# PKU-VCL-Geometry/GeoSplatting

Hardware: AMD Instinct MI355X
Metric: fwd+bwd views/sec at 2M Gaussians, 800x800 (higher is better)
Workload: dtype f32

## Files before the change

### geosplatting_amd/csrc/gs_segsort_dev.h

```cpp
#pragma once
#include <stdint.h>

#ifndef GS_SEGSORT_FN
#define GS_SEGSORT_FN __device__ __forceinline__
#endif

typedef unsigned long long gs_u64;

template <bool PAD>
GS_SEGSORT_FN int gs_seg_phys(int i) { return PAD ? i + (i >> 5) : i; }

template <bool F64>
GS_SEGSORT_FN gs_u64 gs_seg_inf() { return F64 ? 0x7ff0000000000000ull : ~0ull; }

template <bool F64>
GS_SEGSORT_FN void gs_seg_cx(gs_u64& a, gs_u64& b)
{
#if defined(__HIP_DEVICE_COMPILE__)
    if (F64) {
        const double x = __builtin_bit_cast(double, a), y = __builtin_bit_cast(double, b);
        double lo, hi;
        asm("v_min_f64 %0, %1, %2" : "=v"(lo) : "v"(x), "v"(y));
        asm("v_max_f64 %0, %1, %2" : "=v"(hi) : "v"(x), "v"(y));
        a = __builtin_bit_cast(gs_u64, lo); b = __builtin_bit_cast(gs_u64, hi);
        return;
    }
#endif
    const gs_u64 lo = a < b ? a : b, hi = a < b ? b : a;
    a = lo; b = hi;
}

template <int F, bool PAD, bool F64, bool GUARD>
GS_SEGSORT_FN void gs_seg_first(gs_u64* buf, int n, int P, int tid, int nthreads)
{
    constexpr int R = 1 << F;
    for (int v = tid; v < (P >> F); v += nthreads) {
        const int base = v << F;
        if (base >= n) break;
        gs_u64 e[R];
#pragma unroll
        for (int r = 0; r < R; ++r) e[r] = (!GUARD || base + r < n) ? buf[gs_seg_phys<PAD>(base + r)] : gs_seg_inf<F64>();
#pragma unroll
        for (int lgk = 1; lgk <= F; ++lgk) {
#pragma unroll
            for (int r = 0; r < R; ++r)
                if (r < (r ^ ((1 << lgk) - 1))) gs_seg_cx<F64>(e[r], e[r ^ ((1 << lgk) - 1)]);
#pragma unroll
            for (int s = lgk - 2; s >= 0; --s) {
#pragma unroll
                for (int r = 0; r < R; ++r)
                    if ((r & (1 << s)) == 0) gs_seg_cx<F64>(e[r], e[r | (1 << s)]);
            }
        }
#pragma unroll
        for (int r = 0; r < R; ++r) if (!GUARD || base + r < n) buf[gs_seg_phys<PAD>(base + r)] = e[r];
    }
}

template <int G, bool PAD, bool F64, bool GUARD>
GS_SEGSORT_FN void gs_seg_group(gs_u64* buf, int n, int P, int a, bool flip, int tid, int nthreads)
{
    constexpr int R = 1 << G, H = R >> 1;
    const int jmask = (1 << a) - 1;
    for (int v = tid; v < (P >> G); v += nthreads) {
        const int base = ((v >> a) << (a + G)) | (v & jmask);
        if (base >= n) break;
        const int base2 = flip ? (base ^ jmask) : base;
        gs_u64 e[R];
#pragma unroll
        for (int r = 0; r < R; ++r) {
            const int i = (r >= H ? base2 : base) + (r << a);
            e[r] = (!GUARD || i < n) ? buf[gs_seg_phys<PAD>(i)] : gs_seg_inf<F64>();
        }
        if (flip) {
#pragma unroll
            for (int r = 0; r < H; ++r) gs_seg_cx<F64>(e[r], e[R - 1 - r]);
        } else {
#pragma unroll
            for (int r = 0; r < H; ++r) gs_seg_cx<F64>(e[r], e[r + H]);
        }
#pragma unroll
        for (int s = G - 2; s >= 0; --s) {
#pragma unroll
            for (int r = 0; r < R; ++r)
                if ((r & (1 << s)) == 0) gs_seg_cx<F64>(e[r], e[r | (1 << s)]);
        }
#pragma unroll
        for (int r = 0; r < R; ++r) {
            const int i = (r >= H ? base2 : base) + (r << a);
            if (!GUARD || i < n) buf[gs_seg_phys<PAD>(i)] = e[r];
        }
    }
}

template <int GMAX, bool PAD, bool F64, bool GUARD>
GS_SEGSORT_FN void gs_seg_group_n(int g, gs_u64* buf, int n, int P, int a, bool flip, int tid, int nthreads)
{
    if (g == GMAX) gs_seg_group<GMAX, PAD, F64, GUARD>(buf, n, P, a, flip, tid, nthreads);
    else if constexpr (GMAX > 1) gs_seg_group_n<GMAX - 1, PAD, F64, GUARD>(g, buf, n, P, a, flip, tid, nthreads);
}

#define GS_SEG_SORT_BODY(GMAX, PAD, F64, GUARD, buf, n, P, tid, nthreads, BARRIER)                           \
    do {                                                                                                     \
        gs_seg_first<GMAX, PAD, F64, GUARD>(buf, n, P, tid, nthreads);                                       \
        BARRIER;                                                                                             \
        for (int k_ = 2 << (GMAX), lgk_ = (GMAX) + 1; k_ <= (P); k_ <<= 1, ++lgk_) {                         \
            int rem_ = lgk_;                                                                                 \
            bool flip_ = true;                                                                               \
            while (rem_ > 0) {                                                                               \
                const int g_ = flip_ ? ((rem_ - 1) % (GMAX)) + 1 : (GMAX);                                   \
                gs_seg_group_n<GMAX, PAD, F64, GUARD>(g_, buf, n, P, rem_ - g_, flip_, tid, nthreads);       \
                BARRIER;                                                                                     \
                rem_ -= g_;                                                                                  \
                flip_ = false;                                                                               \
            }                                                                                                \
        }                                                                                                    \
    } while (0)
```

### geosplatting_amd/csrc/gs_sort.hip

```cpp
#include "gs_common.h"
#include "gs_segsort_dev.h"

#include <cstdlib>
#include <cstring>

#define RS_THREADS 256
#define RS_WAVES 4
#define RS_ITEMS 8
#define RS_TILE (RS_THREADS * RS_ITEMS)
#define RS_WCHUNK (64 * RS_ITEMS)

typedef unsigned long long u64;

static int tile_bits(int tile_w, int tile_h)
{
    unsigned n = (unsigned)(tile_w * tile_h);
    int b = 0;
    while (n > 1) { n >>= 1; ++b; }
    return b + 1;
}

struct PairItem { u64 key; int32_t val; };
struct PairIn {
    const u64* keys; const int32_t* vals;
    __device__ __forceinline__ PairItem load(int64_t i) const { return PairItem{ keys[i], vals[i] }; }
};
struct PairOut {
    u64* keys; int32_t* vals;
    __device__ __forceinline__ void store(int64_t i, const PairItem& it) const { keys[i] = it.key; vals[i] = it.val; }
};
struct PairDigit {
    int shift; unsigned mask;
    __device__ __forceinline__ unsigned operator()(const PairItem& it) const { return (unsigned)(it.key >> shift) & mask; }
};

struct U2In {
    const uint2* p;
    __device__ __forceinline__ uint2 load(int64_t i) const { return p[i]; }
};
struct U2Out {
    uint2* p;
    __device__ __forceinline__ void store(int64_t i, const uint2& it) const { p[i] = it; }
};
struct DepthIn {
    const float* depths;
    __device__ __forceinline__ uint2 load(int64_t i) const { return make_uint2(__float_as_uint(depths[i]), (unsigned)i); }
};
struct XDigit {
    int shift; unsigned mask;
    __device__ __forceinline__ unsigned operator()(const uint2& it) const { return (it.x >> shift) & mask; }
};
struct FinalTiles {
    int32_t* tile_ids; int32_t* flatten_ids;
    __device__ __forceinline__ void store(int64_t i, const uint2& it) const
    {
        flatten_ids[i] = (int32_t)it.y;
        tile_ids[i] = (int32_t)it.x;
    }
};
struct FinalOut {
    u64* isect_ids; int32_t* flatten_ids; const float* depths;
    __device__ __forceinline__ void store(int64_t i, const uint2& it) const
    {
        flatten_ids[i] = (int32_t)it.y;
        isect_ids[i] = ((u64)it.x << 32) | (u64)__float_as_uint(depths[it.y]);
    }
};

template <typename Item, typename In, typename Digit>
__global__ void __launch_bounds__(RS_THREADS)
radix_hist_kernel(GsCount nc, In in, Digit digit, int nbins, int nblocks, unsigned* __restrict__ table)
{
    const int64_t n = gs_count(nc);
    __shared__ unsigned hist[256];
    hist[threadIdx.x] = 0u;
    __syncthreads();
    const int64_t base = (int64_t)blockIdx.x * RS_TILE;
#pragma unroll 4
    for (int k = 0; k < RS_ITEMS; ++k) {
        const int64_t i = base + (int64_t)k * RS_THREADS + threadIdx.x;
        if (i < n) atomicAdd(&hist[digit(in.load(i))], 1u);
    }
    __syncthreads();
    if ((int)threadIdx.x < nbins) table[(size_t)threadIdx.x * nblocks + blockIdx.x] = hist[threadIdx.x];
}

__global__ void __launch_bounds__(256)
radix_rowscan_kernel(int nblocks, unsigned* __restrict__ table, unsigned* __restrict__ row_total)
{
    __shared__ unsigned wsum[4];
    unsigned* row = table + (size_t)blockIdx.x * nblocks;
    const int lane = threadIdx.x & 63, wave = threadIdx.x >> 6;
    unsigned carry = 0u;
    for (int i0 = 0; i0 < nblocks; i0 += 256) {
        const int i = i0 + threadIdx.x;
        const unsigned v = i < nblocks ? row[i] : 0u;
        unsigned incl = v;
        incl = gs_wave_incl_scan(incl);
        if (lane == 63) wsum[wave] = incl;
        __syncthreads();
        unsigned before = 0u, all = 0u;
        for (int w = 0; w < 4; ++w) { if (w < wave) before += wsum[w]; all += wsum[w]; }
        if (i < nblocks) row[i] = carry + before + incl - v;
        carry += all;
        __syncthreads();
    }
    if (threadIdx.x == 0) row_total[blockIdx.x] = carry;
}

template <typename Item, typename In, typename Digit, typename Out, int NBITS>
__global__ void __launch_bounds__(RS_THREADS)
radix_scatter_kernel(GsCount nc, In in, Digit digit, int nblocks, const unsigned* __restrict__ table,
                     const unsigned* __restrict__ row_total, Out out)
{
    const int64_t n = gs_count(nc);
    constexpr int NB = 1 << NBITS;
    __shared__ unsigned cnt[RS_WAVES][NB];
    __shared__ unsigned dstart[NB];
    __shared__ unsigned gbase[NB];
    __shared__ Item stage[RS_TILE];
    const int lane = threadIdx.x & 63, wave = threadIdx.x >> 6;
    for (int i = threadIdx.x; i < RS_WAVES * NB; i += RS_THREADS) (&cnt[0][0])[i] = 0u;
    __syncthreads();
    const int64_t bbase = (int64_t)blockIdx.x * RS_TILE;
    const int64_t wbase = bbase + (int64_t)wave * RS_WCHUNK;
    const int n_here = (n - bbase) < RS_TILE ? (int)((n - bbase) > 0 ? (n - bbase) : 0) : RS_TILE;
    const u64 lane_lt = (1ull << lane) - 1ull;
    Item item[RS_ITEMS];
    unsigned dig[RS_ITEMS];
    unsigned rank[RS_ITEMS];
#pragma unroll
    for (int k = 0; k < RS_ITEMS; ++k) {
        const int64_t i = wbase + (int64_t)k * 64 + lane;
        const bool valid = i < n;
        if (valid) item[k] = in.load(i);
        const unsigned d = valid ? digit(item[k]) : 0u;
        u64 m = __ballot(valid);
#pragma unroll
        for (int b = 0; b < NBITS; ++b) {
            const bool bit = (d >> b) & 1u;
            const u64 bal = __ballot(bit);
            m &= bit ? bal : ~bal;
        }
        const unsigned old = cnt[wave][d];
        __builtin_amdgcn_wave_barrier();
        const unsigned r = __popcll(m & lane_lt);
        if (valid && r == 0u) cnt[wave][d] = old + (unsigned)__popcll(m);
        __builtin_amdgcn_fence(__ATOMIC_RELEASE, "wavefront");
        __builtin_amdgcn_wave_barrier();
        __builtin_amdgcn_fence(__ATOMIC_ACQUIRE, "wavefront");
        dig[k] = d;
        rank[k] = old + r;
    }
    __syncthreads();
    {
// ... 167 lines not shown

extern "C" int gs_isect_bin(int V, const float* means2d, const int32_t* radii, const float* depths,
                            const int32_t* tiles_per_gauss, int64_t n_isects, int tile_size, int tile_w, int tile_h,
                            int64_t* isect_ids_sorted, int32_t* flatten_ids_sorted, void* ws, size_t ws_bytes, void* stream)
{
    (void)tiles_per_gauss;
    return isect_bin_impl(V, means2d, radii, depths, n_isects, nullptr, tile_size, tile_w, tile_h, isect_ids_sorted, flatten_ids_sorted,
                          ws, ws_bytes, stream, nullptr);
}

extern "C" int gs_isect_bin_cap(int V_cap, const float* means2d, const int32_t* radii, const float* depths, const int64_t* counts_dev,
                                int64_t n_isects_cap, int tile_size, int tile_w, int tile_h, int64_t* isect_ids_sorted,
                                int32_t* flatten_ids_sorted, void* ws, size_t ws_bytes, int64_t* status_dev, void* stream)
{
    GS_CHECK_ARG(counts_dev != nullptr && status_dev != nullptr, "counts_dev / status_dev must not be NULL");
    hipLaunchKernelGGL(capacity_check_kernel, dim3(1), dim3(64), 0, (hipStream_t)stream, (const long long*)counts_dev, (long long)V_cap,
                       (long long)n_isects_cap, (long long*)status_dev);
    GS_CHECK_LAUNCH();
    return isect_bin_impl(V_cap, means2d, radii, depths, n_isects_cap, (const long long*)counts_dev, tile_size, tile_w, tile_h,
                          isect_ids_sorted, flatten_ids_sorted, ws, ws_bytes, stream, nullptr);
}

extern "C" int gs_isect_bin_tiles_cap(int V_cap, const float* means2d, const int32_t* radii, const float* depths, const int64_t* counts_dev,
                                      int64_t n_isects_cap, int tile_size, int tile_w, int tile_h, int32_t* tile_ids_sorted,
                                      int32_t* flatten_ids_sorted, void* ws, size_t ws_bytes, int64_t* status_dev, void* stream)
{
    GS_CHECK_ARG(counts_dev != nullptr && status_dev != nullptr && tile_ids_sorted != nullptr, "counts_dev / status_dev / tile_ids_sorted must not be NULL");
    hipLaunchKernelGGL(capacity_check_kernel, dim3(1), dim3(64), 0, (hipStream_t)stream, (const long long*)counts_dev, (long long)V_cap,
                       (long long)n_isects_cap, (long long*)status_dev);
    GS_CHECK_LAUNCH();
    return isect_bin_impl(V_cap, means2d, radii, depths, n_isects_cap, (const long long*)counts_dev, tile_size, tile_w, tile_h,
                          nullptr, flatten_ids_sorted, ws, ws_bytes, stream, tile_ids_sorted);
}

struct KeyIn {
    const unsigned* keys;
    __device__ __forceinline__ uint2 load(int64_t i) const { return make_uint2(keys[i], (unsigned)i); }
};
#define BF_HIST_MAX 8192

__global__ void __launch_bounds__(256)
bin_setup_kernel(unsigned* __restrict__ state, int n_state_words,
                 const long long* __restrict__ counts, long long v_cap, long long i_cap, long long* __restrict__ status)
{
    const int i = blockIdx.x * blockDim.x + threadIdx.x, stride = gridDim.x * blockDim.x;
    for (int k = i; k < n_state_words; k += stride) state[k] = 0u;
    if (i == 0 && counts != nullptr && status != nullptr) {
        const long long V = counts[0], I = counts[1];
        if (V > v_cap || I > i_cap) {
            status[0] = GS_ENOSPC;
            if (I > status[1]) status[1] = I;
            if (V > status[2]) status[2] = V;
        }
    }
}

#define BF_VALID (1ull << 63)
#define BF_SPIN_LIMIT (1 << 22)

__global__ void __launch_bounds__(EM_THREADS)
emit_chained_kernel(GsCount vc, const uint2* __restrict__ order, const uint2* __restrict__ rect, unsigned* __restrict__ ctrl,
                    u64* __restrict__ desc, int n_blocks, int tile_w, uint2* __restrict__ items, unsigned item_cap,
                    long long* __restrict__ status )
{
    const int V = (int)gs_count(vc);
    __shared__ unsigned ws[EM_THREADS / 64];
    __shared__ unsigned s_block;
    __shared__ unsigned long long s_base;
    const int lane = threadIdx.x & 63, wave = threadIdx.x >> 6;
    if (threadIdx.x == 0) s_block = atomicAdd(ctrl, 1u);
    __syncthreads();
    const int block = (int)s_block;
    u64* agg = desc; u64* pre = desc + n_blocks;
    const int r0 = block * EM_TILE + (int)threadIdx.x * EM_PER;
    int v[EM_PER]; unsigned c[EM_PER]; uint2 q[EM_PER];
    unsigned mine = 0u;
#pragma unroll
    for (int k = 0; k < EM_PER; ++k) {
        const int r = r0 + k;
        v[k] = r < V ? (int)order[r].y : -1;
        q[k] = v[k] >= 0 ? rect[v[k]] : make_uint2(0u, 0u);
        c[k] = rect_count(q[k]);
        mine += c[k];
    }
    unsigned incl = mine;
    incl = gs_wave_incl_scan(incl);
    if (lane == 63) ws[wave] = incl;
    __syncthreads();
    unsigned before = 0u, total = 0u;
    for (int w = 0; w < EM_THREADS / 64; ++w) { if (w < wave) before += ws[w]; total += ws[w]; }
    if (wave == 0) {
        unsigned long long acc = 0ull;
        if (block > 0) {
            if (lane == 0) __hip_atomic_store(&agg[block], (u64)total | BF_VALID, __ATOMIC_RELAXED, __HIP_MEMORY_SCOPE_AGENT);
            int pos = block - 1;
            bool done = false;
            while (!done) {
                u64 pv[EM_LOOK], av[EM_LOOK];
#pragma unroll
                for (int j = 0; j < EM_LOOK; ++j) {
                    const int idx = pos - 64 * j - lane;
                    pv[j] = av[j] = 0ull;
                    if (idx >= 0) {
                        pv[j] = __hip_atomic_load(&pre[idx], __ATOMIC_RELAXED, __HIP_MEMORY_SCOPE_AGENT);
                        av[j] = __hip_atomic_load(&agg[idx], __ATOMIC_RELAXED, __HIP_MEMORY_SCOPE_AGENT);
                    }
                }
#pragma unroll
                for (int j = 0; j < EM_LOOK; ++j) {
                    if (done) break;
                    const int idx = pos - 64 * j - lane;
                    bool isP = idx < 0;
                    u64 val = 0ull;
                    if (idx >= 0) {
                        int spins = 0;
                        for (;;) {
                            if (pv[j] & BF_VALID) { isP = true; val = pv[j]; break; }
                            if (av[j] & BF_VALID) { val = av[j]; break; }
                            if (++spins > BF_SPIN_LIMIT) { atomicExch(ctrl + 1, 1u); if (status) status[0] = GS_ENOSPC; break; }
                            __builtin_amdgcn_s_sleep(2);
                            pv[j] = __hip_atomic_load(&pre[idx], __ATOMIC_RELAXED, __HIP_MEMORY_SCOPE_AGENT);
                            av[j] = __hip_atomic_load(&agg[idx], __ATOMIC_RELAXED, __HIP_MEMORY_SCOPE_AGENT);
                        }
                    }
                    const u64 pmask = __ballot(isP);
                    const int first = pmask ? __builtin_ctzll(pmask) : 64;
                    if (lane <= first) acc += val & ~BF_VALID;
                    if (pmask) done = true;
                }
                pos -= 64 * EM_LOOK;
            }
        }
        const unsigned long long base = gs_wave_sum_u64(acc);
        if (lane == 0) {
            __hip_atomic_store(&pre[block], (u64)(base + total) | BF_VALID, __ATOMIC_RELAXED, __HIP_MEMORY_SCOPE_AGENT);
            s_base = base;
        }
    }
    __syncthreads();
    unsigned long long cur = s_base + before + incl - mine;
#pragma unroll
    for (int k = 0; k < EM_PER; ++k) {
        if (v[k] < 0 || c[k] == 0u) continue;
        const int x0 = (int)(q[k].x & 0xffffu), y0 = (int)(q[k].x >> 16), x1 = (int)(q[k].y & 0xffffu), y1 = (int)(q[k].y >> 16);
        for (int i = y0; i < y1; ++i)
            for (int j = x0; j < x1; ++j) {
                const unsigned t = (unsigned)(i * tile_w + j);
                if (cur < (unsigned long long)item_cap) items[cur] = make_uint2(t, (unsigned)v[k]);
                ++cur;
            }
    }
}

#define SEG_CLASSES 3
#define SEG_CAP0 2048
#define SEG_CAP1 4096
#define SEG_CAP2 16384
#define SEG_GMAX 4
#define SEG_THREADS(cap) ((cap) >> SEG_GMAX > 1024 ? 1024 : ((cap) >> SEG_GMAX))
#define SEG_BINS 64
static size_t seg_lds_bytes(int cap) { return (size_t)(cap + (cap >> 5) + 1) * sizeof(u64); }

extern "C" int gs_isect_bin_front_classes(int* caps, int max)
{
    const int c[SEG_CLASSES] = { SEG_CAP0, SEG_CAP1, SEG_CAP2 };
    for (int i = 0; i < SEG_CLASSES && i < max; ++i) if (caps) caps[i] = c[i];
    return SEG_CLASSES;
}

struct SegLists { unsigned* count; int32_t* lists; };

__device__ __forceinline__ int seg_class(unsigned len) { return len <= SEG_CAP0 ? 0 : (len <= SEG_CAP1 ? 1 : (len <= SEG_CAP2 ? 2 : 3)); }
__device__ __forceinline__ int seg_bin(unsigned len)
{
    const int l2 = 31 - __clz((int)len);
    const int half = l2 > 0 ? (int)((len >> (l2 - 1)) & 1u) : 0;
    return SEG_BINS - 1 - (2 * l2 + half);
}

__global__ void __launch_bounds__(1024)
tile_offsets_scan_kernel(int n_tiles, const unsigned* __restrict__ tile_counts, GsCount nc, int32_t* __restrict__ offsets, SegLists sl)
{
    __shared__ unsigned wsum[16];
    __shared__ unsigned s_bin[(SEG_CLASSES + 1) * SEG_BINS];
    const unsigned n = (unsigned)gs_count(nc);
    const int lane = threadIdx.x & 63, wave = threadIdx.x >> 6;
    if (sl.count && threadIdx.x < (SEG_CLASSES + 1) * SEG_BINS) s_bin[threadIdx.x] = 0u;
    __syncthreads();
    unsigned carry = 0u;
    for (int i0 = 0; i0 < n_tiles; i0 += 1024) {
        const int i = i0 + threadIdx.x;
        const unsigned v = i < n_tiles ? tile_counts[i] : 0u;
        unsigned incl = v;
        incl = gs_wave_incl_scan(incl);
        if (lane == 63) wsum[wave] = incl;
        __syncthreads();
        unsigned before = 0u, all = 0u;
        for (int w = 0; w < 16; ++w) { if (w < wave) before += wsum[w]; all += wsum[w]; }
        if (i < n_tiles) {
            const unsigned o = carry + before + incl - v;
            const unsigned beg = o < n ? o : n, end = o + v < n ? o + v : n;
            offsets[i] = (int32_t)beg;
            if (sl.count && end > beg) atomicAdd(&s_bin[seg_class(end - beg) * SEG_BINS + seg_bin(end - beg)], 1u);
        }
        carry += all;
        __syncthreads();
    }
    if (!sl.count) return;
    if (wave <= SEG_CLASSES) {
        const unsigned v = s_bin[wave * SEG_BINS + lane];
        const unsigned incl = gs_wave_incl_scan(v);
        s_bin[wave * SEG_BINS + lane] = incl - v;
        if (lane == 63) sl.count[wave] = incl;
    }
    __syncthreads();
    for (int i = threadIdx.x; i < n_tiles; i += 1024) {
        const unsigned beg = (unsigned)offsets[i];
        unsigned end = n;
        if (i + 1 < n_tiles) end = (unsigned)__hip_atomic_load(&offsets[i + 1], __ATOMIC_RELAXED, __HIP_MEMORY_SCOPE_WORKGROUP);
        if (end > beg) {
            const int c = seg_class(end - beg);
            const unsigned pos = atomicAdd(&s_bin[c * SEG_BINS + seg_bin(end - beg)], 1u);
            sl.lists[(size_t)c * n_tiles + pos] = i;
        }
    }
}

#define SC_THREADS 512
#define SC_PER 8
#define SC_TILE (SC_THREADS * SC_PER)

__global__ void __launch_bounds__(SC_THREADS)
bin_scatter_kernel(GsCount vc, const unsigned* __restrict__ keys, const uint2* __restrict__ rects, unsigned key_mask, u64 item_bias, int tile_w, int tile_h,
                   const int32_t* __restrict__ offsets, unsigned* __restrict__ cursor, u64* __restrict__ items, unsigned item_cap)
{
    extern __shared__ unsigned s_pos[];
    const int V = (int)gs_count(vc);
    const int n_tiles = tile_w * tile_h;
    const int s0 = (int)blockIdx.x * SC_TILE + (int)threadIdx.x;
    if ((long long)blockIdx.x * SC_TILE >= V) return;
    for (int t = threadIdx.x; t < n_tiles; t += SC_THREADS) s_pos[t] = 0u;
    unsigned key[SC_PER]; uint2 q[SC_PER];
#pragma unroll
    for (int k = 0; k < SC_PER; ++k) {
        const int v = s0 + k * SC_THREADS;
        const int vv = v < V ? v : V - 1;
        key[k] = keys[vv];
        q[k] = rects[vv];
        if (v >= V) q[k] = make_uint2(0u, 0u);
    }
#pragma unroll
    for (int k = 0; k < SC_PER; ++k) {
        int x1 = (int)(q[k].y & 0xffffu), y1 = (int)(q[k].y >> 16);
        x1 = x1 < tile_w ? x1 : tile_w; y1 = y1 < tile_h ? y1 : tile_h;
        q[k].y = (unsigned)x1 | ((unsigned)y1 << 16);
    }
    __syncthreads();
#pragma unroll
    for (int k = 0; k < SC_PER; ++k) {
        const int x0 = (int)(q[k].x & 0xffffu), y0 = (int)(q[k].x >> 16), x1 = (int)(q[k].y & 0xffffu), y1 = (int)(q[k].y >> 16);
        for (int i = y0; i < y1; ++i)
            for (int j = x0; j < x1; ++j) atomicAdd(&s_pos[i * tile_w + j], 1u);
    }
    __syncthreads();
    for (int t0 = threadIdx.x; t0 < n_tiles; t0 += 4 * SC_THREADS) {
        unsigned c[4], o[4], b[4];
#pragma unroll
        for (int u = 0; u < 4; ++u) {
            const int t = t0 + u * SC_THREADS;
            c[u] = t < n_tiles ? s_pos[t] : 0u;
            o[u] = c[u] ? (unsigned)offsets[t] : 0u;
        }
#pragma unroll
        for (int u = 0; u < 4; ++u) b[u] = c[u] ? atomicAdd(&cursor[t0 + u * SC_THREADS], c[u]) : 0u;
#pragma unroll
        for (int u = 0; u < 4; ++u) if (c[u]) s_pos[t0 + u * SC_THREADS] = o[u] + b[u];
    }
    __syncthreads();
#pragma unroll
    for (int k = 0; k < SC_PER; ++k) {
        const int x0 = (int)(q[k].x & 0xffffu), y0 = (int)(q[k].x >> 16), x1 = (int)(q[k].y & 0xffffu), y1 = (int)(q[k].y >> 16);
        const u64 item = item_bias | ((u64)(key[k] & key_mask) << 31) | (u64)(unsigned)(s0 + k * SC_THREADS);
        for (int i = y0; i < y1; ++i)
            for (int j = x0; j < x1; ++j) {
                const unsigned pos = atomicAdd(&s_pos[i * tile_w + j], 1u);
                if (pos < item_cap) items[pos] = item;
            }
    }
}

template <int THREADS, bool GLOBAL, bool F64>
__global__ void __launch_bounds__(THREADS)
seg_sort_kernel(const int32_t* __restrict__ list, const unsigned* __restrict__ list_count, int n_tiles, const int32_t* __restrict__ offsets,
                GsCount ic, GsCount vc, u64* items, int32_t* __restrict__ flat)
{
    extern __shared__ u64 s_seg[];
    if (blockIdx.x >= *list_count) return;
    const int t = list[blockIdx.x];
    const int n_all = (int)gs_count(ic);
    const int beg = offsets[t], end = t + 1 < n_tiles ? offsets[t + 1] : n_all;
    const int n = end - beg;
    if (n <= 0) return;
    const long long V = gs_count(vc);
    const unsigned vmax = V > 0 ? (unsigned)(V - 1) : 0u;
    const int tid = threadIdx.x;
    int P = 1 << SEG_GMAX;
    while (P < n) P <<= 1;
    u64* buf = GLOBAL ? items + beg : s_seg;
    if (!GLOBAL) {
        for (int i = tid; i < P; i += THREADS) s_seg[gs_seg_phys<true>(i)] = i < n ? items[beg + i] : gs_seg_inf<F64>();
        __syncthreads();
    }
    GS_SEG_SORT_BODY(SEG_GMAX, !GLOBAL, F64, GLOBAL, buf, n, P, tid, THREADS, __syncthreads());
    for (int i = tid; i < n; i += THREADS) {
        const unsigned slot = (unsigned)buf[gs_seg_phys<!GLOBAL>(i)] & 0x7fffffffu;
        flat[beg + i] = (int32_t)(slot < vmax ? slot : vmax);
    }
}

__global__ void __launch_bounds__(256)
bin_offsets_tiles_kernel(GsCount nc, const int32_t* __restrict__ tiles, int n_tiles, int32_t* __restrict__ offsets)
{
    const int64_t n = gs_count(nc);
    const int64_t i = (int64_t)blockIdx.x * blockDim.x + threadIdx.x;
    if (n == 0 && i == 0)
        for (int t = 0; t < n_tiles; ++t) offsets[t] = 0;
    if (i >= n) return;
    const int cur = tiles[i];
    if (i == 0) {
        for (int t = 0; t <= cur && t < n_tiles; ++t) offsets[t] = 0;
    } else {
        const int prev = tiles[i - 1];
        for (int t = prev + 1; t <= cur && t < n_tiles; ++t) offsets[t] = (int32_t)i;
    }
    if (i == n - 1)
        for (int t = cur + 1; t < n_tiles; ++t) offsets[t] = (int32_t)n;
}


static size_t tf_state_words(int n_tiles) { return (size_t)n_tiles + SEG_CLASSES + 1; }
static size_t tf_ws_bytes(int64_t n_isects, int n_tiles)
{
    return align256(tf_state_words(n_tiles) * 4) + align256((size_t)(SEG_CLASSES + 1) * n_tiles * 4) + align256((size_t)n_isects * 8) + 256;
}
static size_t bf_radix_ws_bytes(size_t v, size_t n)
{
    return table_bytes((int64_t)(v > n ? v : n)) + 2 * align256(v * 8) + 2 * align256(n * 8) + bf_state_bytes((int)v) + align256(n * 4) + 256;
}

extern "C" size_t gs_isect_bin_front_ws_bytes(int V, int64_t n_isects, int tile_w, int tile_h)
{
    const size_t v = V > 0 ? (size_t)V : 1, n = n_isects > 0 ? (size_t)n_isects : 1;
    const int64_t n_tiles = (int64_t)tile_w * tile_h;
    if (n_tiles > 0 && n_tiles <= BF_HIST_MAX) return tf_ws_bytes((int64_t)n, (int)n_tiles);
    return bf_radix_ws_bytes(v, n);
}

static int bin_front_tile_first(int V, const uint32_t* depth_keys, const uint32_t* tile_rects, const uint32_t* tile_counts,
                                const int64_t* counts_dev, int64_t n_isects, int key_bits, int tile_w, int tile_h, int32_t* flatten_ids_sorted,
                                int32_t* isect_offsets, void* ws, int64_t* status_dev, hipStream_t s)
{
    const int n_tiles = tile_w * tile_h;
    const GsCount vc{ (long long)V, (const long long*)counts_dev }, ic{ (long long)n_isects, counts_dev ? (const long long*)counts_dev + 1 : nullptr };
    char* p = (char*)ws;
    unsigned* cursor = (unsigned*)p;
    unsigned* class_count = cursor + n_tiles; p += align256(tf_state_words(n_tiles) * 4);
    int32_t* lists = (int32_t*)p; p += align256((size_t)(SEG_CLASSES + 1) * n_tiles * 4);
    u64* items = (u64*)p;
    const int n_state_words = (int)tf_state_words(n_tiles);
    hipLaunchKernelGGL(bin_setup_kernel, dim3(gs_cdiv(n_state_words, 256) < 64 ? gs_cdiv(n_state_words, 256) : 64), dim3(256), 0, s, cursor,
                       n_state_words, (const long long*)counts_dev, (long long)V, (long long)n_isects, (long long*)status_dev);
    GS_CHECK_LAUNCH();
    hipLaunchKernelGGL(tile_offsets_scan_kernel, dim3(1), dim3(1024), 0, s, n_tiles, (const unsigned*)tile_counts, ic, isect_offsets,
                       SegLists{ class_count, lists });
    GS_CHECK_LAUNCH();
    const bool f64 = key_bits == 24;
    hipLaunchKernelGGL(bin_scatter_kernel, dim3(gs_cdiv(V, SC_TILE)), dim3(SC_THREADS), (size_t)n_tiles * 4, s, vc,
                       (const unsigned*)depth_keys, (const uint2*)tile_rects, f64 ? 0xffffffu : 0xffffffffu, f64 ? (1ull << 62) : 0ull, tile_w, tile_h,
                       (const int32_t*)isect_offsets, cursor, items, (unsigned)n_isects);
    GS_CHECK_LAUNCH();
    GS_CHECK_HIP(hipFuncSetAttribute((const void*)seg_sort_kernel<SEG_THREADS(SEG_CAP2), false, false>, hipFuncAttributeMaxDynamicSharedMemorySize, (int)seg_lds_bytes(SEG_CAP2)));
    GS_CHECK_HIP(hipFuncSetAttribute((const void*)seg_sort_kernel<SEG_THREADS(SEG_CAP2), false, true>, hipFuncAttributeMaxDynamicSharedMemorySize, (int)seg_lds_bytes(SEG_CAP2)));
    const int caps[SEG_CLASSES + 1] = { 0, SEG_CAP0, SEG_CAP1, SEG_CAP2 };
    for (int c = 0; c <= SEG_CLASSES; ++c) {
        const int64_t most = n_isects / (caps[c] + 1);
        const int grid = (int)(most < n_tiles ? most : n_tiles);
        if (grid == 0) continue;
        const int32_t* list = lists + (size_t)c * n_tiles;
#define SEG_LAUNCH1(T, G, F, LDS) hipLaunchKernelGGL((seg_sort_kernel<T, G, F>), dim3(grid), dim3(T), LDS, s, list, (const unsigned*)(class_count + c), n_tiles, \
                                                     (const int32_t*)isect_offsets, ic, vc, items, flatten_ids_sorted)
#define SEG_LAUNCH(T, G, LDS) do { if (f64) SEG_LAUNCH1(T, G, true, LDS); else SEG_LAUNCH1(T, G, false, LDS); } while (0)
        if (c == 0) SEG_LAUNCH(SEG_THREADS(SEG_CAP0), false, seg_lds_bytes(SEG_CAP0));
        else if (c == 1) SEG_LAUNCH(SEG_THREADS(SEG_CAP1), false, seg_lds_bytes(SEG_CAP1));
        else if (c == 2) SEG_LAUNCH(SEG_THREADS(SEG_CAP2), false, seg_lds_bytes(SEG_CAP2));
        else SEG_LAUNCH(1024, true, 0);
#undef SEG_LAUNCH
#undef SEG_LAUNCH1
        GS_CHECK_LAUNCH();
    }
    return GS_OK;
}

extern "C" int gs_isect_bin_front(int V_cap, const uint32_t* depth_keys, const uint32_t* tile_rects, const uint32_t* tile_counts,
                                  const int64_t* counts_dev, int64_t n_isects_cap, int key_bits, int tile_w, int tile_h, int32_t* flatten_ids_sorted,
                                  int32_t* isect_offsets, void* ws, size_t ws_bytes, int64_t* status_dev, void* stream)
{
    const int V = V_cap;
    const int64_t n_isects = n_isects_cap;
    GS_CHECK_ARG(V >= 0 && n_isects >= 0 && tile_w > 0 && tile_h > 0 && (key_bits == 24 || key_bits == 32), "bad sizes or key width");
    GS_CHECK_ARG(n_isects < (1ll << 31), "n_isects must fit int32");
    GS_CHECK_ARG((int64_t)tile_w * tile_h < (1ll << 24) && tile_w < 65536 && tile_h < 65536, "tile grid too large");
    GS_CHECK_ARG(isect_offsets != nullptr && (counts_dev == nullptr || status_dev != nullptr), "null argument");
    hipStream_t s = (hipStream_t)stream;
    const int n_tiles = tile_w * tile_h;
    if (V == 0 || n_isects == 0) { GS_CHECK_HIP(gs_zero_async(isect_offsets, sizeof(int32_t) * (size_t)n_tiles, s)); return GS_OK; }
    GS_CHECK_ARG(depth_keys != nullptr && tile_rects != nullptr && flatten_ids_sorted != nullptr && ws != nullptr, "null argument");
    if (tile_counts != nullptr && n_tiles <= BF_HIST_MAX) {
        if (ws_bytes < tf_ws_bytes(n_isects, n_tiles)) { gs_set_error("gs_isect_bin_front: workspace too small"); return GS_ENOSPC; }
        return bin_front_tile_first(V, depth_keys, tile_rects, tile_counts, counts_dev, n_isects, key_bits, tile_w, tile_h, flatten_ids_sorted,
                                    isect_offsets, ws, status_dev, s);
    }
    if (ws_bytes < bf_radix_ws_bytes((size_t)V, (size_t)n_isects)) { gs_set_error("gs_isect_bin_front: workspace too small for the radix path (no tile_counts)"); return GS_ENOSPC; }
    const GsCount vc{ (long long)V, (const long long*)counts_dev }, ic{ (long long)n_isects, counts_dev ? (const long long*)counts_dev + 1 : nullptr };
    char* p = (char*)ws;
    unsigned* table = (unsigned*)p; p += table_bytes((int64_t)V > n_isects ? (int64_t)V : n_isects);
    uint2* da = (uint2*)p; p += align256((size_t)V * 8);
    uint2* db = (uint2*)p; p += align256((size_t)V * 8);
    uint2* ia = (uint2*)p; p += align256((size_t)n_isects * 8);
    uint2* ib = (uint2*)p; p += align256((size_t)n_isects * 8);
    unsigned* state = (unsigned*)p; p += bf_state_bytes(V);
    int32_t* tile_ids = (int32_t*)p;
    const int eblocks = (V + EM_TILE - 1) / EM_TILE;
    const int n_state_words = (int)(bf_state_bytes(V) / 4);
    hipLaunchKernelGGL(bin_setup_kernel, dim3(gs_cdiv(n_state_words, 256) < 64 ? gs_cdiv(n_state_words, 256) : 64),
                       dim3(256), 0, s, state, n_state_words, (const long long*)counts_dev,
                       (long long)V_cap, (long long)n_isects_cap, (long long*)status_dev);
    GS_CHECK_LAUNCH();
    int rc = radix_pass<uint2>(vc, KeyIn{ depth_keys }, XDigit{ 0, 255u }, U2Out{ da }, 8, table, s);
    if (rc != GS_OK) return rc;
    rc = radix_pass<uint2>(vc, U2In{ da }, XDigit{ 8, 255u }, U2Out{ db }, 8, table, s);
    if (rc != GS_OK) return rc;
    rc = radix_pass<uint2>(vc, U2In{ db }, XDigit{ 16, 255u }, U2Out{ da }, 8, table, s);
    if (rc != GS_OK) return rc;
    const uint2* order = da;
    if (key_bits == 32) {
        rc = radix_pass<uint2>(vc, U2In{ da }, XDigit{ 24, 255u }, U2Out{ db }, 8, table, s);
        if (rc != GS_OK) return rc;
        order = db;
    }
    unsigned* ctrl = state; u64* desc = (u64*)((char*)state + 16);
    hipLaunchKernelGGL(emit_chained_kernel, dim3(eblocks), dim3(EM_THREADS), 0, s, vc, order, (const uint2*)tile_rects, ctrl, desc,
                       eblocks + 1, tile_w, ia, (unsigned)n_isects, (long long*)status_dev);
    GS_CHECK_LAUNCH();
    int tb = 0;
    while ((1 << tb) < n_tiles) ++tb;
    if (tb < 1) tb = 1;
    const int npass = (tb + 7) / 8, width = (tb + npass - 1) / npass;
    uint2* src = ia; uint2* dst = ib;
    for (int pass = 0; pass < npass; ++pass) {
        const int shift = pass * width;
        const int nbits = (tb - shift) < width ? (tb - shift) : width;
        if (pass == npass - 1)
            rc = radix_pass<uint2>(ic, U2In{ src }, XDigit{ shift, (1u << nbits) - 1u }, FinalTiles{ tile_ids, flatten_ids_sorted }, nbits, table, s);
        else
            rc = radix_pass<uint2>(ic, U2In{ src }, XDigit{ shift, (1u << nbits) - 1u }, U2Out{ dst }, nbits, table, s);
        if (rc != GS_OK) return rc;
        uint2* t = src; src = dst; dst = t;
    }
    hipLaunchKernelGGL(bin_offsets_tiles_kernel, dim3(gs_cdiv(n_isects, 256)), dim3(256), 0, s, ic, tile_ids, n_tiles, isect_offsets);
    GS_CHECK_LAUNCH();
    return GS_OK;
}

static int isect_bin_impl(int V, const float* means2d, const int32_t* radii, const float* depths, int64_t n_isects,
                          const long long* counts_dev, int tile_size, int tile_w, int tile_h, int64_t* isect_ids_sorted,
                          int32_t* flatten_ids_sorted, void* ws, size_t ws_bytes, void* stream, int32_t* tile_ids_sorted)
{
    const GsCount vc{ (long long)V, counts_dev }, ic{ (long long)n_isects, counts_dev ? counts_dev + 1 : nullptr };
    GS_CHECK_ARG(V >= 0 && n_isects >= 0 && tile_size > 0 && tile_w > 0 && tile_h > 0, "bad sizes");
    GS_CHECK_ARG(n_isects < (1ll << 31), "n_isects must fit int32");
    GS_CHECK_ARG((int64_t)tile_w * tile_h < (1ll << 24), "more than 2^24 tiles");
    if (V == 0 || n_isects == 0) return GS_OK;
    GS_CHECK_ARG(ws != nullptr, "workspace must not be NULL");
    if (ws_bytes < gs_isect_bin_ws_bytes(V, n_isects, tile_w, tile_h)) { gs_set_error("gs_isect_bin: workspace too small"); return GS_ENOSPC; }
    hipStream_t s = (hipStream_t)stream;
    char* p = (char*)ws;
    unsigned* table = (unsigned*)p; p += table_bytes((int64_t)V > n_isects ? (int64_t)V : n_isects);
    uint2* da = (uint2*)p; p += align256((size_t)V * 8);
    uint2* db = (uint2*)p; p += align256((size_t)V * 8);
    uint2* rect = (uint2*)p; p += align256((size_t)V * 8);
    const int eblocks = (V + EM_TILE - 1) / EM_TILE;
    unsigned* state = (unsigned*)p; p += bf_state_bytes(V);
    uint2* ia = (uint2*)p; p += align256((size_t)n_isects * 8);
    uint2* ib = (uint2*)p; p += align256((size_t)n_isects * 8);
    int tb = 0;
    while ((1 << tb) < tile_w * tile_h) ++tb;
    if (tb < 1) tb = 1;
    const int npass = (tb + 7) / 8, width = (tb + npass - 1) / npass;
    int rc = GS_OK;
    rc = radix_pass<uint2>(vc, DepthIn{ depths }, XDigit{ 0, 255u }, U2Out{ da }, 8, table, s);
    if (rc != GS_OK) return rc;
    rc = radix_pass<uint2>(vc, U2In{ da }, XDigit{ 8, 255u }, U2Out{ db }, 8, table, s);
    if (rc != GS_OK) return rc;
    rc = radix_pass<uint2>(vc, U2In{ db }, XDigit{ 16, 255u }, U2Out{ da }, 8, table, s);
    if (rc != GS_OK) return rc;
    rc = radix_pass<uint2>(vc, U2In{ da }, XDigit{ 24, 255u }, U2Out{ db }, 8, table, s);
    if (rc != GS_OK) return rc;
    GS_CHECK_ARG(tile_w < 65536 && tile_h < 65536, "tile grid too large");
    hipLaunchKernelGGL(tile_rect_kernel, dim3(gs_cdiv(V, 256)), dim3(256), 0, s, vc, means2d, radii, tile_size, tile_w, tile_h, rect);
    GS_CHECK_LAUNCH();
    {
        const int n_state_words = (int)(bf_state_bytes(V) / 4);
        hipLaunchKernelGGL(bin_setup_kernel, dim3(gs_cdiv(n_state_words, 256) < 64 ? gs_cdiv(n_state_words, 256) : 64), dim3(256), 0, s, state,
                           n_state_words, (const long long*)nullptr, 0ll, 0ll, (long long*)nullptr);
        GS_CHECK_LAUNCH();
        hipLaunchKernelGGL(emit_chained_kernel, dim3(eblocks), dim3(EM_THREADS), 0, s, vc, (const uint2*)db, (const uint2*)rect, state,
                           (u64*)((char*)state + 16), eblocks + 1, tile_w, ia, (unsigned)n_isects, (long long*)nullptr);
        GS_CHECK_LAUNCH();
    }
    uint2* src = ia; uint2* dst = ib;
    for (int pass = 0; pass < npass; ++pass) {
        const int shift = pass * width;
        const int nbits = (tb - shift) < width ? (tb - shift) : width;
        if (pass == npass - 1 && tile_ids_sorted != nullptr)
            rc = radix_pass<uint2>(ic, U2In{ src }, XDigit{ shift, (1u << nbits) - 1u },
                                   FinalTiles{ tile_ids_sorted, flatten_ids_sorted }, nbits, table, s);
        else if (pass == npass - 1)
            rc = radix_pass<uint2>(ic, U2In{ src }, XDigit{ shift, (1u << nbits) - 1u },
                                   FinalOut{ (u64*)isect_ids_sorted, flatten_ids_sorted, depths }, nbits, table, s);
        else
            rc = radix_pass<uint2>(ic, U2In{ src }, XDigit{ shift, (1u << nbits) - 1u }, U2Out{ dst }, nbits, table, s);
        if (rc != GS_OK) return rc;
        uint2* t = src; src = dst; dst = t;
    }
    return GS_OK;
}
```

Measured before the change: 756.5.

## Sort long tile segments in LDS-sized chunks with a persistent chunked kernel

Replaces the three size classes (2K/4K/16K LDS sorts plus a global-memory bitonic fallback) with two lists. Short segments keep the single-block LDS sort. Longer ones go to a persistent grid-stride kernel that sorts 4096-element chunks in LDS and does only the cross-chunk bitonic stages in global memory, reloading each chunk for the in-chunk stages. This aims to cut the fully global sort path for long tiles and the 16K-entry LDS footprint that limits occupancy. The cost is more global passes for medium segments (4K–16K) that previously sorted entirely in LDS, and a grid capped at 2 blocks per CU.

```diff
diff --git a/geosplatting_amd/csrc/gs_segsort_dev.h b/geosplatting_amd/csrc/gs_segsort_dev.h
--- a/geosplatting_amd/csrc/gs_segsort_dev.h
+++ b/geosplatting_amd/csrc/gs_segsort_dev.h
@@ -31,10 +31,10 @@
 }
 
 template <int F, bool PAD, bool F64, bool GUARD>
-GS_SEGSORT_FN void gs_seg_first(gs_u64* buf, int n, int P, int tid, int nthreads)
+GS_SEGSORT_FN void gs_seg_first(gs_u64* buf, int n, unsigned P, int tid, int nthreads)
 {
     constexpr int R = 1 << F;
-    for (int v = tid; v < (P >> F); v += nthreads) {
+    for (int v = tid; v < (int)(P >> F); v += nthreads) {
         const int base = v << F;
         if (base >= n) break;
         gs_u64 e[R];
@@ -58,11 +58,11 @@
 }
 
 template <int G, bool PAD, bool F64, bool GUARD>
-GS_SEGSORT_FN void gs_seg_group(gs_u64* buf, int n, int P, int a, bool flip, int tid, int nthreads)
+GS_SEGSORT_FN void gs_seg_group(gs_u64* buf, int n, unsigned P, int a, bool flip, int tid, int nthreads)
 {
     constexpr int R = 1 << G, H = R >> 1;
     const int jmask = (1 << a) - 1;
-    for (int v = tid; v < (P >> G); v += nthreads) {
+    for (int v = tid; v < (int)(P >> G); v += nthreads) {
         const int base = ((v >> a) << (a + G)) | (v & jmask);
         if (base >= n) break;
         const int base2 = flip ? (base ^ jmask) : base;
@@ -94,25 +94,93 @@
 }
 
 template <int GMAX, bool PAD, bool F64, bool GUARD>
-GS_SEGSORT_FN void gs_seg_group_n(int g, gs_u64* buf, int n, int P, int a, bool flip, int tid, int nthreads)
+GS_SEGSORT_FN void gs_seg_group_n(int g, gs_u64* buf, int n, unsigned P, int a, bool flip, int tid, int nthreads)
 {
     if (g == GMAX) gs_seg_group<GMAX, PAD, F64, GUARD>(buf, n, P, a, flip, tid, nthreads);
     else if constexpr (GMAX > 1) gs_seg_group_n<GMAX - 1, PAD, F64, GUARD>(g, buf, n, P, a, flip, tid, nthreads);
 }
 
-#define GS_SEG_SORT_BODY(GMAX, PAD, F64, GUARD, buf, n, P, tid, nthreads, BARRIER)                           \
+#define GS_SEG_SORT_BODY_E(GMAX, PAD, F64, GUARD, buf, n, P, tid, nthreads, EACH, BARRIER)                   \
     do {                                                                                                     \
-        gs_seg_first<GMAX, PAD, F64, GUARD>(buf, n, P, tid, nthreads);                                       \
+        EACH gs_seg_first<GMAX, PAD, F64, GUARD>(buf, n, P, tid, nthreads);                                  \
         BARRIER;                                                                                             \
-        for (int k_ = 2 << (GMAX), lgk_ = (GMAX) + 1; k_ <= (P); k_ <<= 1, ++lgk_) {                         \
+        for (int lgk_ = (GMAX) + 1; lgk_ < 32 && (1u << lgk_) <= (unsigned)(P); ++lgk_) {                   \
             int rem_ = lgk_;                                                                                 \
             bool flip_ = true;                                                                               \
             while (rem_ > 0) {                                                                               \
                 const int g_ = flip_ ? ((rem_ - 1) % (GMAX)) + 1 : (GMAX);                                   \
-                gs_seg_group_n<GMAX, PAD, F64, GUARD>(g_, buf, n, P, rem_ - g_, flip_, tid, nthreads);       \
+                EACH gs_seg_group_n<GMAX, PAD, F64, GUARD>(g_, buf, n, P, rem_ - g_, flip_, tid, nthreads);  \
                 BARRIER;                                                                                     \
                 rem_ -= g_;                                                                                  \
                 flip_ = false;                                                                               \
             }                                                                                                \
         }                                                                                                    \
     } while (0)
+#define GS_SEG_SORT_BODY(GMAX, PAD, F64, GUARD, buf, n, P, tid, nthreads, BARRIER)                           \
+    GS_SEG_SORT_BODY_E(GMAX, PAD, F64, GUARD, buf, n, P, tid, nthreads, , BARRIER)
+
+template <int LGC>
+constexpr int gs_seg_chunk_words() { return (1 << LGC) + (1 << LGC >> 5) + 1; }
+
+template <bool F64>
+GS_SEGSORT_FN void gs_seg_chunk_load(gs_u64* lds, const gs_u64* src, int cnt, int P, int tid, int nthreads)
+{
+    for (int i = tid; i < P; i += nthreads) lds[gs_seg_phys<true>(i)] = i < cnt ? src[i] : gs_seg_inf<F64>();
+}
+
+GS_SEGSORT_FN void gs_seg_chunk_store(const gs_u64* lds, gs_u64* dst, int cnt, int tid, int nthreads)
+{
+    for (int i = tid; i < cnt; i += nthreads) dst[i] = lds[gs_seg_phys<true>(i)];
+}
+
+GS_SEGSORT_FN void gs_seg_chunk_emit(const gs_u64* lds, int32_t* dst, int cnt, unsigned vmax, int tid, int nthreads)
+{
+    for (int i = tid; i < cnt; i += nthreads) {
+        const unsigned slot = (unsigned)lds[gs_seg_phys<true>(i)] & 0x7fffffffu;
+        dst[i] = (int32_t)(slot < vmax ? slot : vmax);
+    }
+}
+
+#define GS_SEG_CHUNKED_BODY(GMAX, LGC, F64, seg, lds, n, out, vmax, tid, nthreads, EACH, BARRIER)            \
+    do {                                                                                                     \
+        static_assert((LGC) % (GMAX) == 0 && (LGC) >= (GMAX), "the chunk's bit count must be a multiple of GMAX"); \
+        constexpr int C_ = 1 << (LGC);                                                                       \
+        int lgP_ = (GMAX);                                                                                   \
+        while (lgP_ < 31 && (1ll << lgP_) < (long long)(n)) ++lgP_;                                          \
+        const bool one_ = lgP_ <= (LGC);                                                                     \
+        for (int base_ = 0; base_ < (n); base_ = base_ < (n) - C_ ? base_ + C_ : (n)) { \
+            const int cnt_ = (n) - base_ < C_ ? (n) - base_ : C_;                                            \
+            int Pc_ = 1 << (GMAX);                            \
+            while (Pc_ < cnt_) Pc_ <<= 1;                                                                    \
+            EACH gs_seg_chunk_load<F64>(lds, (seg) + base_, cnt_, Pc_, tid, nthreads);                       \
+            BARRIER;                                                                                         \
+            GS_SEG_SORT_BODY_E(GMAX, true, F64, false, lds, cnt_, Pc_, tid, nthreads, EACH, BARRIER);        \
+            if (one_) { EACH gs_seg_chunk_emit(lds, (out) + base_, cnt_, vmax, tid, nthreads); }             \
+            else { EACH gs_seg_chunk_store(lds, (seg) + base_, cnt_, tid, nthreads); }                       \
+            BARRIER;                                                                                         \
+        }                                                                                                    \
+        const unsigned Pn_ = 1u << lgP_;                                  \
+        for (int lgk_ = (LGC) + 1; lgk_ <= lgP_; ++lgk_) {                                                   \
+            int rem_ = lgk_;                                                                                 \
+            bool flip_ = true;                                                                               \
+            while (rem_ > (LGC)) {                                                                           \
+                const int g_ = flip_ ? ((rem_ - 1) % (GMAX)) + 1 : (GMAX);                                   \
+                EACH gs_seg_group_n<GMAX, false, F64, true>(g_, seg, n, Pn_, rem_ - g_, flip_, tid, nthreads); \
+                BARRIER;                                                                                     \
+                rem_ -= g_;                                                                                  \
+                flip_ = false;                                                                               \
+            }                                                                                                \
+            for (int base_ = 0; base_ < (n); base_ = base_ < (n) - C_ ? base_ + C_ : (n)) { \
+                const int cnt_ = (n) - base_ < C_ ? (n) - base_ : C_;                                        \
+                EACH gs_seg_chunk_load<F64>(lds, (seg) + base_, cnt_, C_, tid, nthreads);                    \
+                BARRIER;                                                                                     \
+                for (int a_ = (LGC) - (GMAX); a_ >= 0; a_ -= (GMAX)) {                                       \
+                    EACH gs_seg_group<GMAX, true, F64, false>(lds, cnt_, C_, a_, false, tid, nthreads);      \
+                    BARRIER;                                                                                 \
+                }                                                                                            \
+                if (lgk_ == lgP_) { EACH gs_seg_chunk_emit(lds, (out) + base_, cnt_, vmax, tid, nthreads); } \
+                else { EACH gs_seg_chunk_store(lds, (seg) + base_, cnt_, tid, nthreads); }                   \
+                BARRIER;                                                                                     \
+            }                                                                                                \
+        }                                                                                                    \
+    } while (0)
diff --git a/geosplatting_amd/csrc/gs_sort.hip b/geosplatting_amd/csrc/gs_sort.hip
--- a/geosplatting_amd/csrc/gs_sort.hip
+++ b/geosplatting_amd/csrc/gs_sort.hip
@@ -1,6 +1,7 @@
 #include "gs_common.h"
 #include "gs_segsort_dev.h"
 
+#include <atomic>
 #include <cstdlib>
 #include <cstring>
 
@@ -474,25 +475,30 @@
     }
 }
 
-#define SEG_CLASSES 3
+#define SEG_LISTS 2
 #define SEG_CAP0 2048
-#define SEG_CAP1 4096
-#define SEG_CAP2 16384
+#define SEG_LG_CHUNK 12
+#define SEG_CHUNK (1 << SEG_LG_CHUNK)
 #define SEG_GMAX 4
-#define SEG_THREADS(cap) ((cap) >> SEG_GMAX > 1024 ? 1024 : ((cap) >> SEG_GMAX))
+#define SEG_THREADS(cap) ((cap) >> SEG_GMAX)
 #define SEG_BINS 64
-static size_t seg_lds_bytes(int cap) { return (size_t)(cap + (cap >> 5) + 1) * sizeof(u64); }
+#define SEG_LDS_MAX 33808
+static constexpr size_t seg_lds_bytes(int cap) { return (size_t)(cap + (cap >> 5) + 1) * sizeof(u64); }
+static_assert(SEG_LG_CHUNK % SEG_GMAX == 0, "the in-chunk groups of a long merge must be full groups");
+static_assert(seg_lds_bytes(SEG_CHUNK) <= SEG_LDS_MAX && seg_lds_bytes(SEG_CHUNK) == gs_seg_chunk_words<SEG_LG_CHUNK>() * sizeof(u64),
+              "a chunk must fit beside the compositor's blocks");
+static_assert(SEG_THREADS(SEG_CHUNK) <= 256 && SEG_CAP0 <= SEG_CHUNK, "resource shape of the sort workgroups");
 
 extern "C" int gs_isect_bin_front_classes(int* caps, int max)
 {
-    const int c[SEG_CLASSES] = { SEG_CAP0, SEG_CAP1, SEG_CAP2 };
-    for (int i = 0; i < SEG_CLASSES && i < max; ++i) if (caps) caps[i] = c[i];
-    return SEG_CLASSES;
+    const int c[4] = { SEG_CAP0, SEG_CHUNK, 2 * SEG_CHUNK, 4 * SEG_CHUNK };
+    for (int i = 0; i < 4 && i < max; ++i) if (caps) caps[i] = c[i];
+    return 4;
 }
 
 struct SegLists { unsigned* count; int32_t* lists; };
 
-__device__ __forceinline__ int seg_class(unsigned len) { return len <= SEG_CAP0 ? 0 : (len <= SEG_CAP1 ? 1 : (len <= SEG_CAP2 ? 2 : 3)); }
+__device__ __forceinline__ int seg_list(unsigned len) { return len <= SEG_CAP0 ? 0 : 1; }
 __device__ __forceinline__ int seg_bin(unsigned len)
 {
     const int l2 = 31 - __clz((int)len);
@@ -504,10 +510,10 @@
 tile_offsets_scan_kernel(int n_tiles, const unsigned* __restrict__ tile_counts, GsCount nc, int32_t* __restrict__ offsets, SegLists sl)
 {
     __shared__ unsigned wsum[16];
-    __shared__ unsigned s_bin[(SEG_CLASSES + 1) * SEG_BINS];
+    __shared__ unsigned s_bin[SEG_LISTS * SEG_BINS];
     const unsigned n = (unsigned)gs_count(nc);
     const int lane = threadIdx.x & 63, wave = threadIdx.x >> 6;
-    if (sl.count && threadIdx.x < (SEG_CLASSES + 1) * SEG_BINS) s_bin[threadIdx.x] = 0u;
+    if (sl.count && threadIdx.x < SEG_LISTS * SEG_BINS) s_bin[threadIdx.x] = 0u;
     __syncthreads();
     unsigned carry = 0u;
     for (int i0 = 0; i0 < n_tiles; i0 += 1024) {
@@ -523,13 +529,13 @@
             const unsigned o = carry + before + incl - v;
             const unsigned beg = o < n ? o : n, end = o + v < n ? o + v : n;
             offsets[i] = (int32_t)beg;
-            if (sl.count && end > beg) atomicAdd(&s_bin[seg_class(end - beg) * SEG_BINS + seg_bin(end - beg)], 1u);
+            if (sl.count && end > beg) atomicAdd(&s_bin[seg_list(end - beg) * SEG_BINS + seg_bin(end - beg)], 1u);
         }
         carry += all;
         __syncthreads();
     }
     if (!sl.count) return;
-    if (wave <= SEG_CLASSES) {
+    if (wave < SEG_LISTS) {
         const unsigned v = s_bin[wave * SEG_BINS + lane];
         const unsigned incl = gs_wave_incl_scan(v);
         s_bin[wave * SEG_BINS + lane] = incl - v;
@@ -541,7 +547,7 @@
         unsigned end = n;
         if (i + 1 < n_tiles) end = (unsigned)__hip_atomic_load(&offsets[i + 1], __ATOMIC_RELAXED, __HIP_MEMORY_SCOPE_WORKGROUP);
         if (end > beg) {
-            const int c = seg_class(end - beg);
+            const int c = seg_list(end - beg);
             const unsigned pos = atomicAdd(&s_bin[c * SEG_BINS + seg_bin(end - beg)], 1u);
             sl.lists[(size_t)c * n_tiles + pos] = i;
         }
@@ -611,10 +617,10 @@
     }
 }
 
-template <int THREADS, bool GLOBAL, bool F64>
+template <int THREADS, bool F64>
 __global__ void __launch_bounds__(THREADS)
 seg_sort_kernel(const int32_t* __restrict__ list, const unsigned* __restrict__ list_count, int n_tiles, const int32_t* __restrict__ offsets,
-                GsCount ic, GsCount vc, u64* items, int32_t* __restrict__ flat)
+                GsCount ic, GsCount vc, const u64* __restrict__ items, int32_t* __restrict__ flat)
 {
     extern __shared__ u64 s_seg[];
     if (blockIdx.x >= *list_count) return;
@@ -628,15 +634,32 @@
     const int tid = threadIdx.x;
     int P = 1 << SEG_GMAX;
     while (P < n) P <<= 1;
-    u64* buf = GLOBAL ? items + beg : s_seg;
-    if (!GLOBAL) {
-        for (int i = tid; i < P; i += THREADS) s_seg[gs_seg_phys<true>(i)] = i < n ? items[beg + i] : gs_seg_inf<F64>();
-        __syncthreads();
-    }
-    GS_SEG_SORT_BODY(SEG_GMAX, !GLOBAL, F64, GLOBAL, buf, n, P, tid, THREADS, __syncthreads());
-    for (int i = tid; i < n; i += THREADS) {
-        const unsigned slot = (unsigned)buf[gs_seg_phys<!GLOBAL>(i)] & 0x7fffffffu;
-        flat[beg + i] = (int32_t)(slot < vmax ? slot : vmax);
+    gs_seg_chunk_load<F64>(s_seg, items + beg, n, P, tid, THREADS);
+    __syncthreads();
+    GS_SEG_SORT_BODY(SEG_GMAX, true, F64, false, s_seg, n, P, tid, THREADS, __syncthreads());
+    gs_seg_chunk_emit(s_seg, flat + beg, n, vmax, tid, THREADS);
+}
+
+template <bool F64>
+__global__ void __launch_bounds__(SEG_THREADS(SEG_CHUNK))
+seg_sort_chunked_kernel(const int32_t* __restrict__ list, const unsigned* __restrict__ list_count, int n_tiles, const int32_t* __restrict__ offsets,
+                        GsCount ic, GsCount vc, u64* items, int32_t* __restrict__ flat)
+{
+    extern __shared__ u64 s_seg[];
+    constexpr int THREADS = SEG_THREADS(SEG_CHUNK);
+    const unsigned count = *list_count;
+    const int n_all = (int)gs_count(ic);
+    const long long V = gs_count(vc);
+    const unsigned vmax = V > 0 ? (unsigned)(V - 1) : 0u;
+    const int tid = threadIdx.x;
+    for (unsigned b = blockIdx.x; b < count; b += gridDim.x) {
+        const int t = list[b];
+        const int beg = offsets[t], end = t + 1 < n_tiles ? offsets[t + 1] : n_all;
+        const int n = end - beg;
+        if (n <= 0) continue;
+        u64* seg = items + beg;
+        int32_t* out = flat + beg;
+        GS_SEG_CHUNKED_BODY(SEG_GMAX, SEG_LG_CHUNK, F64, seg, s_seg, n, out, vmax, tid, THREADS, , __syncthreads());
     }
 }
 
@@ -660,10 +683,10 @@
 }
 
 
-static size_t tf_state_words(int n_tiles) { return (size_t)n_tiles + SEG_CLASSES + 1; }
+static size_t tf_state_words(int n_tiles) { return (size_t)n_tiles + SEG_LISTS; }
 static size_t tf_ws_bytes(int64_t n_isects, int n_tiles)
 {
-    return align256(tf_state_words(n_tiles) * 4) + align256((size_t)(SEG_CLASSES + 1) * n_tiles * 4) + align256((size_t)n_isects * 8) + 256;
+    return align256(tf_state_words(n_tiles) * 4) + align256((size_t)SEG_LISTS * n_tiles * 4) + align256((size_t)n_isects * 8) + 256;
 }
 static size_t bf_radix_ws_bytes(size_t v, size_t n)
 {
@@ -678,6 +701,23 @@
     return bf_radix_ws_bytes(v, n);
 }
 
+#define SEG_PER_CU 2
+#define SEG_MAX_DEVICES 64
+static int seg_resident_grid(int* grid)
+{
+    static std::atomic<int> n_cu[SEG_MAX_DEVICES];
+    int dev = 0;
+    GS_CHECK_HIP(hipGetDevice(&dev));
+    int n = dev >= 0 && dev < SEG_MAX_DEVICES ? n_cu[dev].load(std::memory_order_relaxed) : 0;
+    if (n == 0) {
+        GS_CHECK_HIP(hipDeviceGetAttribute(&n, hipDeviceAttributeMultiprocessorCount, dev));
+        if (n <= 0) n = 256;
+        if (dev >= 0 && dev < SEG_MAX_DEVICES) n_cu[dev].store(n, std::memory_order_relaxed);
+    }
+    *grid = SEG_PER_CU * n;
+    return GS_OK;
+}
+
 static int bin_front_tile_first(int V, const uint32_t* depth_keys, const uint32_t* tile_rects, const uint32_t* tile_counts,
                                 const int64_t* counts_dev, int64_t n_isects, int key_bits, int tile_w, int tile_h, int32_t* flatten_ids_sorted,
                                 int32_t* isect_offsets, void* ws, int64_t* status_dev, hipStream_t s)
@@ -686,40 +726,40 @@
     const GsCount vc{ (long long)V, (const long long*)counts_dev }, ic{ (long long)n_isects, counts_dev ? (const long long*)counts_dev + 1 : nullptr };
     char* p = (char*)ws;
     unsigned* cursor = (unsigned*)p;
-    unsigned* class_count = cursor + n_tiles; p += align256(tf_state_words(n_tiles) * 4);
-    int32_t* lists = (int32_t*)p; p += align256((size_t)(SEG_CLASSES + 1) * n_tiles * 4);
+    unsigned* list_counts = cursor + n_tiles; p += align256(tf_state_words(n_tiles) * 4);
+    int32_t* lists = (int32_t*)p; p += align256((size_t)SEG_LISTS * n_tiles * 4);
     u64* items = (u64*)p;
     const int n_state_words = (int)tf_state_words(n_tiles);
     hipLaunchKernelGGL(bin_setup_kernel, dim3(gs_cdiv(n_state_words, 256) < 64 ? gs_cdiv(n_state_words, 256) : 64), dim3(256), 0, s, cursor,
                        n_state_words, (const long long*)counts_dev, (long long)V, (long long)n_isects, (long long*)status_dev);
     GS_CHECK_LAUNCH();
     hipLaunchKernelGGL(tile_offsets_scan_kernel, dim3(1), dim3(1024), 0, s, n_tiles, (const unsigned*)tile_counts, ic, isect_offsets,
-                       SegLists{ class_count, lists });
+                       SegLists{ list_counts, lists });
     GS_CHECK_LAUNCH();
     const bool f64 = key_bits == 24;
     hipLaunchKernelGGL(bin_scatter_kernel, dim3(gs_cdiv(V, SC_TILE)), dim3(SC_THREADS), (size_t)n_tiles * 4, s, vc,
                        (const unsigned*)depth_keys, (const uint2*)tile_rects, f64 ? 0xffffffu : 0xffffffffu, f64 ? (1ull << 62) : 0ull, tile_w, tile_h,
                        (const int32_t*)isect_offsets, cursor, items, (unsigned)n_isects);
     GS_CHECK_LAUNCH();
-    GS_CHECK_HIP(hipFuncSetAttribute((const void*)seg_sort_kernel<SEG_THREADS(SEG_CAP2), false, false>, hipFuncAttributeMaxDynamicSharedMemorySize, (int)seg_lds_bytes(SEG_CAP2)));
-    GS_CHECK_HIP(hipFuncSetAttribute((const void*)seg_sort_kernel<SEG_THREADS(SEG_CAP2), false, true>, hipFuncAttributeMaxDynamicSharedMemorySize, (int)seg_lds_bytes(SEG_CAP2)));
-    const int caps[SEG_CLASSES + 1] = { 0, SEG_CAP0, SEG_CAP1, SEG_CAP2 };
-    for (int c = 0; c <= SEG_CLASSES; ++c) {
-        const int64_t most = n_isects / (caps[c] + 1);
-        const int grid = (int)(most < n_tiles ? most : n_tiles);
-        if (grid == 0) continue;
-        const int32_t* list = lists + (size_t)c * n_tiles;
-#define SEG_LAUNCH1(T, G, F, LDS) hipLaunchKernelGGL((seg_sort_kernel<T, G, F>), dim3(grid), dim3(T), LDS, s, list, (const unsigned*)(class_count + c), n_tiles, \
-                                                     (const int32_t*)isect_offsets, ic, vc, items, flatten_ids_sorted)
-#define SEG_LAUNCH(T, G, LDS) do { if (f64) SEG_LAUNCH1(T, G, true, LDS); else SEG_LAUNCH1(T, G, false, LDS); } while (0)
-        if (c == 0) SEG_LAUNCH(SEG_THREADS(SEG_CAP0), false, seg_lds_bytes(SEG_CAP0));
-        else if (c == 1) SEG_LAUNCH(SEG_THREADS(SEG_CAP1), false, seg_lds_bytes(SEG_CAP1));
-        else if (c == 2) SEG_LAUNCH(SEG_THREADS(SEG_CAP2), false, seg_lds_bytes(SEG_CAP2));
-        else SEG_LAUNCH(1024, true, 0);
+    const int grid0 = (int)(n_isects < n_tiles ? n_isects : n_tiles);
+#define SEG_LAUNCH(K, GRID, T, LDS, C) hipLaunchKernelGGL(K, dim3(GRID), dim3(T), LDS, s, (const int32_t*)(lists + (size_t)(C) * n_tiles),      \
+                                                          (const unsigned*)(list_counts + (C)), n_tiles, (const int32_t*)isect_offsets, ic, vc, items, \
+                                                          flatten_ids_sorted)
+    if (f64) SEG_LAUNCH((seg_sort_kernel<SEG_THREADS(SEG_CAP0), true>), grid0, SEG_THREADS(SEG_CAP0), seg_lds_bytes(SEG_CAP0), 0);
+    else SEG_LAUNCH((seg_sort_kernel<SEG_THREADS(SEG_CAP0), false>), grid0, SEG_THREADS(SEG_CAP0), seg_lds_bytes(SEG_CAP0), 0);
+    GS_CHECK_LAUNCH();
+    int resident = 0;
+    const int rc = seg_resident_grid(&resident);
+    if (rc != GS_OK) return rc;
+    const int64_t most = n_isects / (SEG_CAP0 + 1);
+    int grid = (int)(most < n_tiles ? most : n_tiles);
+    if (grid > resident) grid = resident;
+    if (grid > 0) {
+        if (f64) SEG_LAUNCH(seg_sort_chunked_kernel<true>, grid, SEG_THREADS(SEG_CHUNK), seg_lds_bytes(SEG_CHUNK), 1);
+        else SEG_LAUNCH(seg_sort_chunked_kernel<false>, grid, SEG_THREADS(SEG_CHUNK), seg_lds_bytes(SEG_CHUNK), 1);
+        GS_CHECK_LAUNCH();
+    }
 #undef SEG_LAUNCH
-#undef SEG_LAUNCH1
-        GS_CHECK_LAUNCH();
-    }
     return GS_OK;
 }
 
```

New measurement: 755.6. Within noise of the previous version (-0.1%).
